# kostas1515/iif

Hardware: AMD Instinct MI355X
Metric: images/sec ResNet50+IIF ImageNet-LT bs=256/GPU (higher is better)
Workload: dtype bf16

## Files before the change

### iif_amd/_lib.py

```python
import ctypes
import os

import torch

_HERE = os.path.dirname(os.path.abspath(__file__))
LIB_PATH = os.environ.get("IIF_AMD_LIB") or os.path.join(_HERE, "csrc", "libiif_amd.so")

IIF_F32, IIF_BF16 = 0, 1
VARIANT_CODE = {"raw": 0, "smooth": 1, "rel": 2, "normit": 3, "gombit": 4, "base2": 5, "base10": 6}
_ERR = {-1: "IIF_EINVAL (bad argument)", -2: "IIF_EUNSUPPORTED (shape/alignment)", -3: "IIF_ELAUNCH (HIP error)"}

_c = ctypes
_P, _I, _L, _F = _c.c_void_p, _c.c_int, _c.c_int64, _c.c_float

SIGNATURES = {
    "iif_build_table": [_P, _I, _I, _I, _P],
    "iif_set_cu_budget": [_I],
    "iif_get_cu_budget": [],
    "iif_ce_fwd_bwd": [_P, _I, _L, _P, _P, _P, _F, _P, _P, _L, _F, _I, _I, _P, _P, _P, _L, _P, _P, _P],
    "iif_sigmoid_focal_fwd_bwd": [_P, _I, _L, _P, _P, _F, _P, _F, _I, _F, _F, _I, _I, _P, _P, _P, _L, _P, _P, _P],
    "iif_scale_logits": [_P, _I, _L, _P, _I, _I, _P, _L, _P],
    "iif_softmax": [_P, _I, _L, _P, _I, _I, _P, _L, _P],
    "iif_topk_hits": [_P, _I, _L, _P, _P, _I, _I, _P, _I, _P, _P],
    "iif_eval_accumulate": [_P, _I, _L, _P, _P, _I, _I, _P, _I, _P, _I, _P, _P, _P, _P],
    "iif_scale_by_device_scalar": [_P, _I, _L, _P, _P, _P],
    "iif_mix_rows": [_P, _I, _P, _F, _I, _L, _P, _P],
    "iif_conv_igemm": [_P, _P, _P, _P, _P, _P, _P],
    "iif_conv_wgrad": [_P, _P, _P, _P, _P, _L, _I, _P],
    "iif_conv_igemm_bnstats": [_P, _P, _P, _P, _P, _P, _P, _L, _P, _P],
    "iif_bn_finalize_stats": [_P, _I, _L, _I, _P, _P, _F, _F, _P, _P, _P, _P, _L, _P],
    "iif_bn_finalize_stats_fused": [_P, _I, _L, _I, _P, _P, _F, _F, _P, _P, _P, _P, _L, _P, _P],
    "iif_bn_finalize_stats_sums": [_P, _I, _L, _I, _P, _P, _F, _F, _P, _P, _P, _P, _L, _P, _P, _I, _I, _P, _P],
    "iif_bn_backward_partials_fused": [_P, _P, _P, _I, _L, _I, _P, _P, _P, _I, _P, _P, _P, _P, _L, _P, _P],
    "iif_bn_partial_sums": [_P, _I, _I, _P, _P],
    "iif_bn_stats_sums": [_P, _I, _L, _I, _P, _P, _L, _P],
    "iif_bn_backward_sums": [_P, _P, _P, _P, _I, _L, _I, _P, _P, _P, _L, _P],
    "iif_bn_backward_apply_sums": [_P, _P, _P, _P, _I, _L, _I, _P, _P, _P, _P, _c.c_double, _P, _P, _P, _P, _P, _P],
    "iif_bn_workspace_bytes": [_L, _I],
    "iif_bn_forward_stats": [_P, _I, _L, _I, _P, _P, _F, _F, _P, _P, _P, _P, _L, _P],
    "iif_bn_apply": [_P, _I, _L, _I, _P, _P, _P, _I, _P, _P, _P],
    "iif_bn_backward": [_P, _P, _P, _P, _I, _L, _I, _P, _P, _P, _P, _P, _P, _P, _L, _P],
    "iif_maxpool_forward": [_P, _I, _I, _I, _I, _I, _I, _I, _I, _P, _P, _P],
    "iif_maxpool_backward": [_P, _P, _I, _I, _I, _I, _I, _I, _I, _I, _P, _P],
# ... 179 lines not shown
```

### iif_amd/csrc/conv_wgrad.hip

```cpp
#include <stdlib.h>
#include <type_traits>

#include "common.h"
#ifndef IIF_WG_AUX_X
#define IIF_WG_AUX_X 0
#endif
#ifndef IIF_WG_AUX_Y
#define IIF_WG_AUX_Y 0
#endif

namespace {

struct WgArgs {
    const unsigned char* x; const unsigned char* dy; float* out;
    int N, Hs, Ws, Cs, Hd, Wd, Cd, R, S, sshift, pad, ldw, M, K;
    int ktiles, ntiles, steps_per_split, nsteps, nsplits;
    int xpitch, ypitch, groups;
    int64_t slab;
};

template <typename T> struct WT;
template <> struct WT<unsigned short> {
    static constexpr int PE = 8, ROWS = 32;
    static constexpr int pitch(int cols) { return cols * 2 + 32; }
// ... 421 lines not shown
}

struct W1Args {
    const unsigned char* x; const unsigned char* dy; float* out;
    int M, Cs, Cd, ldw, ktiles, ntiles, steps_per_split, nsteps, nsplits;
    int64_t slab;
    const unsigned char* dy2; int Cd1, Cd2;
};

template <int OFF> __device__ __forceinline__ s16x4 tr_read_at(unsigned a) {
    s16x4 v;
    asm volatile("ds_read_b64_tr_b16 %0, %1 offset:%2" : "=v"(v) : "v"(a), "n"(OFF) : "memory");
    return v;
}

template <int BC, int BNW, int NWV>
__device__ __forceinline__ void wgrad1x1_body(const W1Args& a, unsigned x_bytes, unsigned dy_bytes) {
    constexpr int NWN = BNW / 64, WK = NWV / NWN, CW = BC / WK, KJ = CW / 16;
    using SX = Swz<unsigned short, BNW>;
    using SY = Swz<unsigned short, BC>;
    constexpr int RBX = SX::RB, RBY = SY::RB;
    constexpr int XB = 32 * RBX, YB = 32 * RBY, STAGE = XB + YB;
    constexpr int NPX = XB / 1024, NPY = YB / 1024;
    constexpr bool YPAD = NPY < NWV;
    constexpr int NIX = NPX / NWV, NIY = YPAD ? 1 : NPY / NWV, LPS = NIX + NIY;
    constexpr int LPRX = RBX / 16, RPIX = 64 / LPRX, LPRY = RBY / 16, RPIY = 64 / LPRY;
    constexpr unsigned OOB = 0xfffffff0u;
    static_assert(NIX >= 1 && NIY >= 1 && NIX * NWV == NPX && (YPAD || NIY * NWV == NPY) && KJ >= 1, "tile geometry");
    static_assert(2 * STAGE + 16 * RBY < 65536 && 2 * STAGE + 16 * RBX < 65536, "fragment reads use 16-bit immediates");
    __shared__ __attribute__((aligned(1024))) unsigned char smem[3 * STAGE + (YPAD ? 1024 : 0)];

    const int tid = threadIdx.x, lane = tid & 63;
// ... 13 lines not shown
    const bool second = a.dy2 != nullptr && k0 >= a.Cd1;
    const int ycols = a.dy2 == nullptr ? a.Cd : (second ? a.Cd2 : a.Cd1);
    const int yk0 = second ? k0 - a.Cd1 : k0;
    const auto rs_y = __builtin_amdgcn_make_buffer_rsrc(const_cast<unsigned char*>(second ? a.dy2 : a.dy), 0,
                                                        second ? (unsigned)a.M * (unsigned)a.Cd2 * 2u : dy_bytes, 0x00020000);

    unsigned offx[NIX], incx[NIX], offy[NIY], incy[NIY];
#pragma unroll
    for (int i = 0; i < NIX; ++i) {
        const int r = RPIX * (NIX * wave + i) + lane / LPRX;
        const int col = n0 + SX::logical(lane % LPRX, r) * 8;
        const bool ok = col < a.Cs;
        offx[i] = ok ? ((unsigned)(step0 * 32 + r) * (unsigned)a.Cs + (unsigned)col) * 2u : OOB;
        incx[i] = ok ? 64u * (unsigned)a.Cs : 0u;
    }
#pragma unroll
    for (int i = 0; i < NIY; ++i) {
        const int r = RPIY * (NIY * wave + i) + lane / LPRY;
        const int col = yk0 + SY::logical(lane % LPRY, r) * 8;
        const bool ok = col < ycols && (!YPAD || wave < NPY);
        offy[i] = ok ? ((unsigned)(step0 * 32 + r) * (unsigned)ycols + (unsigned)col) * 2u : OOB;
        incy[i] = ok ? 64u * (unsigned)ycols : 0u;
    }
    auto issue = [&](auto stage_c) {
        constexpr int S = decltype(stage_c)::value;
#pragma unroll
        for (int i = 0; i < NIX; ++i) {
            __builtin_amdgcn_raw_ptr_buffer_load_lds(rs_x, (lds_void_w*)(smem + S * STAGE + (NIX * wave + i) * 1024), 16, offx[i], 0, 0, IIF_WG_AUX_X);
            offx[i] += incx[i];
        }
#pragma unroll
        for (int i = 0; i < NIY; ++i) {
            unsigned char* dst = smem + S * STAGE + XB + (NIY * wave + i) * 1024;
            if (YPAD && wave >= NPY) dst = smem + 3 * STAGE;
            __builtin_amdgcn_raw_ptr_buffer_load_lds(rs_y, (lds_void_w*)dst, 16, offy[i], 0, 0, IIF_WG_AUX_Y);
            offy[i] += incy[i];
        }
    };

    const int g = lane >> 4, li = lane & 15, q = li >> 2, pp = li & 3;
    unsigned xo[4], yo[KJ];
    const unsigned sbase = (unsigned)(unsigned long long)(lds_cu8*)smem;
#pragma unroll
    for (int ni = 0; ni < 4; ++ni) xo[ni] = sbase + (unsigned)SX::addr(4 * g + q, (wn * 64 + ni * 16 + 4 * pp) * 2);
// ... 52 lines not shown
        const int k = k0 + wk * CW + kj * 16 + li;
        if (k >= a.Cd) continue;
#pragma unroll
        for (int ni = 0; ni < 4; ++ni) {
            const int n = n0 + wn * 64 + ni * 16 + g * 4;
            if (n >= a.Cs) continue;
            *reinterpret_cast<f32x4*>(out + (int64_t)k * a.ldw + n) = acc[ni][kj];
        }
    }
}

__global__ void __launch_bounds__(512) wgrad1x1_256x128_kernel(W1Args a, unsigned xb, unsigned yb) { wgrad1x1_body<256, 128, 8>(a, xb, yb); }
__global__ void __launch_bounds__(256) wgrad1x1_128x128_kernel(W1Args a, unsigned xb, unsigned yb) { wgrad1x1_body<128, 128, 4>(a, xb, yb); }
__global__ void __launch_bounds__(256) wgrad1x1_64x128_kernel(W1Args a, unsigned xb, unsigned yb) { wgrad1x1_body<64, 128, 4>(a, xb, yb); }
__global__ void __launch_bounds__(256) wgrad1x1_64x64_kernel(W1Args a, unsigned xb, unsigned yb) { wgrad1x1_body<64, 64, 4>(a, xb, yb); }
__global__ void __launch_bounds__(512) wgrad1x1_64x256_kernel(W1Args a, unsigned xb, unsigned yb) { wgrad1x1_body<64, 256, 8>(a, xb, yb); }

struct WgHaloArgs {
    const unsigned char* x; const unsigned char* dy; float* out;
    int N, H, W, Cs, Cd, ldw;
    int ci_tiles, co_tiles, steps_per_split, nsteps, nsplits, HB;
    int grouped;
    int64_t slab;
};

template <int XB, int YB, int D>
__global__ void __launch_bounds__(256) conv3x3_wgrad_halo_kernel(WgHaloArgs a, unsigned x_bytes, unsigned dy_bytes) {
    constexpr int RB = 128;
    constexpr int XR = 32 * XB, YR = 32 * YB;
    constexpr unsigned OOB = 0xfffffff0u;
// ... 118 lines not shown
    }
#endif

    float* out = a.out + (int64_t)split * a.slab;
#pragma unroll
    for (int kj = 0; kj < 4; ++kj) {
        const int k = co0 + kj * 16 + li;
#pragma unroll
        for (int tap = 0; tap < 9; ++tap) {
            const int n = a.grouped ? tap * 64 + wave * 16 + g * 4 : tap * a.Cs + ci0 + wave * 16 + g * 4;
            *reinterpret_cast<f32x4*>(out + (int64_t)k * a.ldw + n) = acc[tap][kj];
        }
    }
}

struct WgStemArgs {
    const unsigned char* x; const unsigned char* dy; float* out;
    int N, H, W, ldw, steps_per_split, nsteps, nsplits, LB, LEAD;
    int64_t slab;
};

__global__ void __launch_bounds__(256) conv4x4_s2d_wgrad_kernel(WgStemArgs a, unsigned x_bytes, unsigned dy_bytes) {
    constexpr int XRB = 32, YRB = 128;
    constexpr int XR = 512, YR = 128;
    constexpr int D = 2;
    constexpr unsigned OOB = 0xfffffff0u;
    using SW = Swz<unsigned short, 64>;
    __shared__ __attribute__((aligned(1024))) unsigned char smem[XR * XRB + YR * YRB];
    unsigned char* const XS = smem;
    unsigned char* const YS = smem + XR * XRB;
// ... 182 lines not shown
    if (splits < 1) splits = 1;
    if (splits > h.nsteps) splits = h.nsteps;
    if (splits > 65535) splits = 65535;
    h.steps_per_split = (h.nsteps + splits - 1) / splits;
    splits = (h.nsteps + h.steps_per_split - 1) / h.steps_per_split;
    h.slab = splits > 1 ? slab : 0;
    h.out = splits > 1 ? ws : dw;
    h.nsplits = splits;
    const dim3 grid((unsigned)(tiles * ((splits + 7) / 8) * 8));
    hipLaunchKernelGGL((conv3x3_wgrad_halo_kernel<8, 4, 2>), grid, dim3(256), 0, st, h, (unsigned)x_bytes, (unsigned)dy_bytes);
    IIF_LAUNCH_CHECK();
    if (splits > 1) return reduce_slabs(ws, ws_bytes, splits, slab, a.groups * a.Cd, a.ldw, a.K, dw, st);
    return IIF_OK;
}

inline int launch_wgrad_stem(const WgArgs& a, float* dw, float* ws, int64_t ws_bytes, int splits_req, int64_t x_bytes,
                             int64_t dy_bytes, hipStream_t st) {
    WgStemArgs h{};
    h.x = a.x; h.dy = a.dy; h.N = a.N; h.H = a.Hd; h.W = a.Wd; h.ldw = a.ldw;
    const int Wp = a.Wd + 3;
    h.LB = (2 * Wp + 2 + 31) / 32;
    h.LEAD = h.LB + (31 + Wp + 1) / 32;
    if (h.LEAD + 2 > 14) return -100;
    const int64_t vt = (int64_t)a.N * (a.Hd + 3) * Wp;
    if (vt > 0x7fff0000LL) return -100;
    h.nsteps = (int)((vt + 31) / 32);
    int splits = splits_req;
    if (splits <= 0) {
        const int per_cu = 2;
        splits = 256 * per_cu / share_of(splits_req);
        const int max_by_work = h.nsteps / 8 > 0 ? h.nsteps / 8 : 1;
        if (splits > max_by_work) splits = max_by_work;
    }
    const int64_t slab = (int64_t)a.Cd * a.ldw;
    const int64_t fit = ws ? ws_bytes / (slab * 4) : 0;
    if (splits > fit) splits = (int)fit;
    if (splits < 1) splits = 1;
    if (splits > h.nsteps) splits = h.nsteps;
    if (splits > 65535) splits = 65535;
    h.steps_per_split = (h.nsteps + splits - 1) / splits;
    splits = (h.nsteps + h.steps_per_split - 1) / h.steps_per_split;
    h.slab = splits > 1 ? slab : 0;
    h.out = splits > 1 ? ws : dw;
    h.nsplits = splits;
    hipLaunchKernelGGL(conv4x4_s2d_wgrad_kernel, dim3((unsigned)(((splits + 7) / 8) * 8)), dim3(256), 0, st, h, (unsigned)x_bytes,
                       (unsigned)dy_bytes);
    IIF_LAUNCH_CHECK();
    if (splits > 1) return reduce_slabs(ws, ws_bytes, splits, slab, a.Cd, a.ldw, a.K, dw, st);
    return IIF_OK;
}

inline int launch_wgrad_1x1(const WgArgs& g, float* dw, float* ws, int64_t ws_bytes, int splits_req, int64_t x_bytes, int64_t dy_bytes,
                            hipStream_t st, const unsigned char* dy2 = nullptr, int cd2 = 0) {
    W1Args a{};
    a.x = g.x; a.dy = g.dy; a.M = g.M; a.Cs = g.Cs; a.Cd = g.Cd; a.ldw = g.ldw;
    a.dy2 = dy2; a.Cd1 = dy2 ? g.Cd - cd2 : g.Cd; a.Cd2 = cd2;
    const int bc = dy2 ? (a.Cd1 % 256 == 0 ? 256 : 128) : ((g.Cd >= 256 && g.Cd % 256 == 0) ? 256 : (g.Cd <= 64 ? 64 : 128));
    static const bool no_wide = getenv("IIF_WGRAD_NO_64X256") != nullptr;
    const int bnw = (g.Cs <= 64 && bc == 64) ? 64 : ((bc == 64 && g.Cs > 128 && g.Cs % 256 == 0 && !no_wide) ? 256 : 128);
    a.ktiles = (g.Cd + bc - 1) / bc;
    a.ntiles = (g.Cs + bnw - 1) / bnw;
    a.nsteps = (g.M + 31) / 32;
    const int tiles = a.ktiles * a.ntiles;
    const int per_cu = bc == 256 ? 1 : (bc == 128 ? 3 : (bnw == 256 ? 2 : 4));
    int splits = splits_req;
    const int64_t slab = (int64_t)g.Cd * g.ldw;
    if (splits <= 0) {
        splits = 256 * per_cu / share_of(splits_req) / tiles;
        if (splits < 1) splits = 1;
        const int max_by_work = a.nsteps / 8 > 0 ? a.nsteps / 8 : 1;
        if (splits > max_by_work) splits = max_by_work;
        static const int small_div = [] { const char* e = getenv("IIF_WGRAD_SMALL_DIV"); return e ? atoi(e) : 2; }();
        static const int gram_div = [] { const char* e = getenv("IIF_WGRAD_GRAM_DIV"); return e ? atoi(e) : 8; }();
        const bool gram = g.x == g.dy && dy2 == nullptr;
        static const int small_kb = [] { const char* e = getenv("IIF_WGRAD_SMALL_KB"); return e ? atoi(e) : 256; }();
        static const int mid_div = [] { const char* e = getenv("IIF_WGRAD_MID_DIV"); return e ? atoi(e) : 2; }();
        const int div = gram ? gram_div : (slab * 4 <= ((int64_t)small_kb << 10) ? small_div : (slab * 4 <= (4 << 20) ? mid_div : 1));
        if (div > 1 && splits > 8) { splits /= div; if (splits < 8) splits = 8; }
    }
    const int64_t fit = ws ? ws_bytes / (slab * 4) : 0;
    if (splits > fit) splits = (int)fit;
    if (splits < 1) splits = 1;
    if (splits > a.nsteps) splits = a.nsteps > 0 ? a.nsteps : 1;
    if (splits > 65535) splits = 65535;
    a.steps_per_split = (a.nsteps + splits - 1) / splits;
    splits = (a.nsteps + a.steps_per_split - 1) / a.steps_per_split;
    if (splits < 1) splits = 1;
    a.slab = splits > 1 ? slab : 0;
    a.out = splits > 1 ? ws : dw;
    a.nsplits = splits;
    const dim3 grid((unsigned)(tiles * ((splits + 7) / 8) * 8));
    const unsigned xb = (unsigned)x_bytes, yb = (unsigned)dy_bytes;
    if (bc == 256) hipLaunchKernelGGL(wgrad1x1_256x128_kernel, grid, dim3(512), 0, st, a, xb, yb);
    else if (bc == 128) hipLaunchKernelGGL(wgrad1x1_128x128_kernel, grid, dim3(256), 0, st, a, xb, yb);
    else if (bnw == 256) hipLaunchKernelGGL(wgrad1x1_64x256_kernel, grid, dim3(512), 0, st, a, xb, yb);
    else if (bnw == 128) hipLaunchKernelGGL(wgrad1x1_64x128_kernel, grid, dim3(256), 0, st, a, xb, yb);
    else hipLaunchKernelGGL(wgrad1x1_64x64_kernel, grid, dim3(256), 0, st, a, xb, yb);
    IIF_LAUNCH_CHECK();
    if (splits > 1) return reduce_slabs(ws, ws_bytes, splits, slab, g.Cd, g.ldw, g.Cs, dw, st);
    return IIF_OK;
}

template <typename T>
int launch_wgrad(WgArgs a, float* dw, float* ws, int64_t ws_bytes, int splits_req, int64_t x_bytes, int64_t dy_bytes,
                 hipStream_t st) {
    constexpr int ROWS = WT<T>::ROWS;
    const bool force_v1 = getenv("IIF_CONV_REGSTAGE") != nullptr;
    const bool dma_ok = !force_v1 && x_bytes < 0x7ffffff0LL && dy_bytes < 0x7ffffff0LL;
    if constexpr (sizeof(T) == 2) {
        const bool shape = a.groups == 1 ? (a.Cs % 64 == 0 && a.Cd % 64 == 0 && a.xpitch == a.Cs && a.ypitch == a.Cd)
                                         : (a.Cs == 64 && a.Cd == 64 && a.ldw >= 576);
        const bool halo = dma_ok && shape && a.R == 3 && a.S == 3 && a.sshift == 0 && a.pad == 1 && a.Hs == a.Hd &&
                          a.Ws == a.Wd && a.Wd + 3 <= 64;
        if (halo) {
            const int rc = launch_wgrad_halo(a, dw, ws, ws_bytes, splits_req, x_bytes, dy_bytes, st);
            if (rc != -100) return rc;
        }
        const bool stem = dma_ok && a.groups == 1 && a.R == 4 && a.S == 4 && a.sshift == 0 && a.pad == 2 && a.Hs == a.Hd &&
                          a.Ws == a.Wd && a.Cs == 16 && a.Cd == 64 && a.xpitch == 16 && a.ypitch == 64;
        if (stem) {
            const int rc = launch_wgrad_stem(a, dw, ws, ws_bytes, splits_req, x_bytes, dy_bytes, st);
            if (rc != -100) return rc;
        }
    }
    if constexpr (sizeof(T) == 2) {
        if (dma_ok && a.R == 1 && a.S == 1 && a.sshift == 0 && a.pad == 0 && a.groups == 1 && a.Hs == a.Hd && a.Ws == a.Wd &&
            a.xpitch == a.Cs && a.ypitch == a.Cd)
            return launch_wgrad_1x1(a, dw, ws, ws_bytes, splits_req, x_bytes, dy_bytes, st);
    }
    bool wide = sizeof(T) == 2 && dma_ok && a.groups == 1 && a.Cd >= 256 && a.Cd % 256 == 0;
    const int bc = wide ? 256 : (a.Cd <= 64 ? 64 : 128);
    a.ktiles = (a.Cd + bc - 1) / bc;
    a.ntiles = (a.K + 127) / 128;
    a.nsteps = (a.M + ROWS - 1) / ROWS;
    const int tiles = a.ktiles * a.ntiles;
    int splits = splits_req;
    if (splits <= 0) {
        const int slots = 256 * (bc == 256 ? 1 : (bc == 128 ? 3 : 4)) / share_of(splits_req);
        splits = slots / (tiles * a.groups);
        if (splits < 1) splits = 1;
        const int max_by_work = a.nsteps / 8 > 0 ? a.nsteps / 8 : 1;
        if (splits > max_by_work) splits = max_by_work;
    }
// ... 19 lines not shown
        if (bc == 64) hipLaunchKernelGGL((conv_wgrad_dma_kernel<T, 64>), grid1d, dim3(256), 0, st, a, xb, yb);
        else if (bc == 256) {
            if constexpr (sizeof(T) == 2) hipLaunchKernelGGL((conv_wgrad_dma_kernel<T, 256, 4>), grid1d, dim3(512), 0, st, a, xb, yb);
        } else hipLaunchKernelGGL((conv_wgrad_dma_kernel<T, 128>), grid1d, dim3(256), 0, st, a, xb, yb);
    } else {
        if (bc == 64) hipLaunchKernelGGL((conv_wgrad_kernel<T, 64>), grid, dim3(256), 0, st, a);
        else hipLaunchKernelGGL((conv_wgrad_kernel<T, 128>), grid, dim3(256), 0, st, a);
    }
    IIF_LAUNCH_CHECK();
    if (splits > 1) return reduce_slabs(ws, ws_bytes, splits, slab, a.groups * a.Cd, a.ldw, a.K, dw, st);
    return IIF_OK;
}

}

extern "C" int iif_conv_wgrad(const iif_conv_desc* d, const void* x, const void* dy, float* dw, void* workspace,
                              int64_t workspace_bytes, int splits, void* stream) {
    if (!d || !x || !dy || !dw) return IIF_EINVAL;
    if (d->n <= 0 || d->hs <= 0 || d->ws <= 0 || d->cs <= 0 || d->hd <= 0 || d->wd <= 0 || d->cd <= 0 ||
        d->r <= 0 || d->s <= 0 || d->pad < 0 || workspace_bytes < 0)
        return IIF_EINVAL;
    if (d->stride != 1 && d->stride != 2) return IIF_EUNSUPPORTED;
    if (d->dtype != IIF_F32 && d->dtype != IIF_BF16) return IIF_EINVAL;
    if (d->transposed) return IIF_EINVAL;
    const int pe = d->dtype == IIF_F32 ? 4 : 8;
    if (d->cs % pe != 0 || d->cd % pe != 0 || d->ldw % 4 != 0 || d->ldw < d->r * d->s * d->cs) return IIF_EUNSUPPORTED;
    if ((reinterpret_cast<uintptr_t>(x) | reinterpret_cast<uintptr_t>(dy) | reinterpret_cast<uintptr_t>(dw) |
         reinterpret_cast<uintptr_t>(workspace)) & 15)
        return IIF_EUNSUPPORTED;
    const int64_t M = (int64_t)d->n * d->hd * d->wd;
    if (M > 0x7fffff00LL || (int64_t)d->n * d->hs * d->ws > 0x7fffff00LL) return IIF_EUNSUPPORTED;
    WgArgs a{};
    a.x = (const unsigned char*)x; a.dy = (const unsigned char*)dy;
    a.N = d->n; a.Hs = d->hs; a.Ws = d->ws; a.Cs = d->cs; a.Hd = d->hd; a.Wd = d->wd; a.Cd = d->cd;
    a.R = d->r; a.S = d->s; a.sshift = d->stride - 1; a.pad = d->pad; a.ldw = d->ldw; a.M = (int)M;
    a.K = d->r * d->s * d->cs;
    a.groups = d->groups > 1 ? d->groups : 1;
    a.xpitch = a.groups * d->cs; a.ypitch = a.groups * d->cd;
    if (a.groups > 65535) return IIF_EUNSUPPORTED;
    hipStream_t st = as_stream(stream);
    const int64_t esz = d->dtype == IIF_F32 ? 4 : 2;
    const int64_t x_bytes = (int64_t)d->n * d->hs * d->ws * a.xpitch * esz, dy_bytes = M * a.ypitch * esz;
    if (d->dtype == IIF_BF16)
        return launch_wgrad<unsigned short>(a, dw, (float*)workspace, workspace_bytes, splits, x_bytes, dy_bytes, st);
    return launch_wgrad<float>(a, dw, (float*)workspace, workspace_bytes, splits, x_bytes, dy_bytes, st);
}

extern "C" int iif_wgrad1x1_stacked(const void* x, const void* dy, const void* dy2, int64_t m, int cs, int cd1, int cd2, int ldw,
                                    float* out, void* workspace, int64_t workspace_bytes, int splits, void* stream) {
    if (!x || !dy || !dy2 || !out || m <= 0 || cs <= 0 || cd1 <= 0 || cd2 <= 0 || workspace_bytes < 0) return IIF_EINVAL;
    if (cs % 8 || cd1 % 128 || cd2 % 8 || ldw % 4 || ldw < cs) return IIF_EUNSUPPORTED;
    if ((reinterpret_cast<uintptr_t>(x) | reinterpret_cast<uintptr_t>(dy) | reinterpret_cast<uintptr_t>(dy2) |
         reinterpret_cast<uintptr_t>(out) | reinterpret_cast<uintptr_t>(workspace)) & 15)
        return IIF_EUNSUPPORTED;
    if (m > 0x7fffff00LL || m * cs * 2 >= 0x7f000000LL || m * cd1 * 2 >= 0x7f000000LL || m * cd2 * 2 >= 0x7f000000LL) return IIF_EUNSUPPORTED;
    WgArgs a{};
    a.x = (const unsigned char*)x; a.dy = (const unsigned char*)dy;
// ... 21 lines not shown
```

### iif_amd/ops.py

```python
import ctypes

import torch

from . import _lib
from ._lib import ConvDesc, check, dtype_code, lib, ptr, require_gpu, stream_ptr


def _desc(n, hs, ws, cs, hd, wd, cd, r, s, stride, pad, transposed, ldw, dtype, dst_dtype, groups=1, w_frag=None):
    kind = 0
    if isinstance(w_frag, tuple):
        w_frag, kind = w_frag
    return ConvDesc(n, hs, ws, cs, hd, wd, cd, r, s, stride, pad, transposed, ldw, dtype, dst_dtype, groups,
                    ptr(w_frag) if w_frag is not None else None, kind)


def conv_out_hw(h, w, r, s, stride, pad):
    return (h + 2 * pad - r) // stride + 1, (w + 2 * pad - s) // stride + 1


def conv_forward(x, w, r, s, stride, pad, out=None, out_dtype=None, bias=None, res=None, groups=1, out_hw=None, w_frag=None):
    require_gpu(x, w, bias, res)
    n, h, wd_, cin = x.shape
    cout, ldw = w.shape
    ho, wo = out_hw or conv_out_hw(h, wd_, r, s, stride, pad)
# ... 88 lines not shown
    n, ho, wo, cout = dy.shape
    cin, ldw = wt.shape
    h, w_ = in_hw
    if out is None:
        out = torch.empty((n, h, w_, cin), dtype=dy.dtype, device=dy.device)
    d = _desc(n, ho, wo, cout // groups, h, w_, cin // groups, r, s, stride, pad, 1, ldw, dtype_code(dy), dtype_code(out),
              groups, w_frag)
    if res_bits is not None:
        check(lib().iif_conv_igemm_masked_res(ctypes.byref(d), ptr(dy), ptr(wt), ptr(out), ptr(res), ptr(res_bits),
                                              stream_ptr()), "iif_conv_igemm_masked_res")
        return out
    check(lib().iif_conv_igemm(ctypes.byref(d), ptr(dy), ptr(wt), ptr(out), ptr(res), 0, stream_ptr()), "iif_conv_igemm(dgrad)")
    return out


def conv_wgrad(x, dy, r, s, stride, pad, ldw=None, out=None, workspace=None, splits=0, groups=1):
    require_gpu(x, dy, out, workspace)
    n, h, w_, cin = x.shape
    _, ho, wo, cout = dy.shape
    k = r * s * (cin // groups)
    ldw = ldw or k
    if out is None:
        out = torch.zeros((cout, ldw), dtype=torch.float32, device=x.device)
    elif not out.is_contiguous() or out.numel() < cout * ldw:
        raise ValueError("conv_wgrad: out must be a contiguous float32 [Cout, ldw] tensor (rows are written with pitch ldw)")
    d = _desc(n, h, w_, cin // groups, ho, wo, cout // groups, r, s, stride, pad, 0, ldw, dtype_code(x), _lib.IIF_F32, groups)
    wsb = 0 if workspace is None else workspace.numel() * workspace.element_size()
    check(lib().iif_conv_wgrad(ctypes.byref(d), ptr(x), ptr(dy), ptr(out), ptr(workspace), wsb, splits, stream_ptr()),
          "iif_conv_wgrad")
    return out
# ... 532 lines not shown
```

### include/iif_amd.h

```cpp
#ifndef IIF_AMD_H
#define IIF_AMD_H

#include <stdint.h>

#ifdef __cplusplus
extern "C" {
#endif

#define IIF_OK 0
#define IIF_EINVAL (-1)
#define IIF_EUNSUPPORTED (-2)
#define IIF_ELAUNCH (-3)

#define IIF_F32 0
#define IIF_BF16 1

#define IIF_RAW 0
#define IIF_SMOOTH 1
#define IIF_REL 2
#define IIF_NORMIT 3
#define IIF_GOMBIT 4
#define IIF_BASE2 5
#define IIF_BASE10 6

// ... 112 lines not shown
    int32_t dst_dtype;
    int32_t groups;
    const void* wgt_frag;
    int32_t wgt_frag_kind;
} iif_conv_desc;

int iif_conv_igemm(const iif_conv_desc* d, const void* src, const void* wgt, void* dst,
                   const void* res, const float* bias, void* stream);

int iif_conv_igemm_bnstats(const iif_conv_desc* d, const void* src, const void* wgt, void* dst,
                           const void* res, const float* bias, float* bn_partial,
                           int64_t bn_partial_floats, int32_t* n_partials, void* stream);

int iif_conv_wgrad(const iif_conv_desc* d, const void* x, const void* dy, float* dw,
                   void* workspace, int64_t workspace_bytes, int splits, void* stream);

int iif_wgrad1x1_stacked(const void* x, const void* dy, const void* dy2, int64_t m, int cs, int cd1, int cd2,
                         int ldw, float* out, void* workspace, int64_t workspace_bytes, int splits,
                         void* stream);

int64_t iif_bn_workspace_bytes(int64_t m, int c);
int iif_bn_forward_stats(const void* x, int dtype, int64_t m, int c, const float* gamma,
                         const float* beta, float eps, float momentum, float* running_mean,
                         float* running_var, float* stats, void* workspace,
                         int64_t workspace_bytes, void* stream);
int iif_bn_apply(const void* x, int dtype, int64_t m, int c, const float* stats,
                 const void* residual, const float* residual_stats, int relu, void* y,
                 uint8_t* relu_bits, void* stream);
typedef struct iif_bn_fold_desc {
    const float* gamma; const float* beta; const float* running_mean; const float* running_var;
// ... 299 lines not shown
```

Before: 15290.

## Add specialized stride-2 weight-gradient kernels for 1x1 and 3x3 convolutions

Adds two new weight-gradient paths for stride-2 convolutions, which previously fell back to the general kernel. The 1x1 path is a gather variant of the 1x1 kernel that walks strided input positions incrementally. The 3x3 path uses a ring buffer over parity planes so the nine taps share LDS data and feed MFMA. It also factors routing into a wgrad_family function with a query API, adding kernel complexity and new edge-case logic for odd spatial sizes.

```diff
diff --git a/iif_amd/_lib.py b/iif_amd/_lib.py
--- a/iif_amd/_lib.py
+++ b/iif_amd/_lib.py
@@ -27,6 +27,7 @@
     "iif_mix_rows": [_P, _I, _P, _F, _I, _L, _P, _P],
     "iif_conv_igemm": [_P, _P, _P, _P, _P, _P, _P],
     "iif_conv_wgrad": [_P, _P, _P, _P, _P, _L, _I, _P],
+    "iif_conv_wgrad_route": [_P],
     "iif_conv_igemm_bnstats": [_P, _P, _P, _P, _P, _P, _P, _L, _P, _P],
     "iif_bn_finalize_stats": [_P, _I, _L, _I, _P, _P, _F, _F, _P, _P, _P, _P, _L, _P],
     "iif_bn_finalize_stats_fused": [_P, _I, _L, _I, _P, _P, _F, _F, _P, _P, _P, _P, _L, _P, _P],
diff --git a/iif_amd/csrc/conv_wgrad.hip b/iif_amd/csrc/conv_wgrad.hip
--- a/iif_amd/csrc/conv_wgrad.hip
+++ b/iif_amd/csrc/conv_wgrad.hip
@@ -459,8 +459,10 @@
     return v;
 }
 
-template <int BC, int BNW, int NWV>
-__device__ __forceinline__ void wgrad1x1_body(const W1Args& a, unsigned x_bytes, unsigned dy_bytes) {
+struct W1Gather { int N, Hs, Ws, Hd, Wd; };
+
+template <int BC, int BNW, int NWV, bool GATHER = false>
+__device__ __forceinline__ void wgrad1x1_body(const W1Args& a, unsigned x_bytes, unsigned dy_bytes, const W1Gather& z = W1Gather{}) {
     constexpr int NWN = BNW / 64, WK = NWV / NWN, CW = BC / WK, KJ = CW / 16;
     using SX = Swz<unsigned short, BNW>;
     using SY = Swz<unsigned short, BC>;
@@ -504,6 +506,29 @@
         offx[i] = ok ? ((unsigned)(step0 * 32 + r) * (unsigned)a.Cs + (unsigned)col) * 2u : OOB;
         incx[i] = ok ? 64u * (unsigned)a.Cs : 0u;
     }
+    int gn[NIX], gh[NIX], gw[NIX];
+    bool gok[NIX];
+    int g_rw = 0, g_rh = 0, g_dn = 0;
+    unsigned g_k0 = 0, g_kc = 0, g_kr = 0;
+    if constexpr (GATHER) {
+        const int dq = 32 / z.Wd;
+        g_rw = 32 - dq * z.Wd; g_rh = dq % z.Hd; g_dn = dq / z.Hd;
+        const unsigned colb = 4u * (unsigned)a.Cs, rowb = colb * (unsigned)z.Ws, imgb = 2u * (unsigned)a.Cs * (unsigned)z.Hs * (unsigned)z.Ws;
+        g_k0 = (unsigned)g_rw * colb + (unsigned)g_rh * rowb + (unsigned)g_dn * imgb;
+        g_kc = rowb - (unsigned)z.Wd * colb;
+        g_kr = imgb - (unsigned)z.Hd * rowb;
+#pragma unroll
+        for (int i = 0; i < NIX; ++i) {
+            const int r = RPIX * (NIX * wave + i) + lane / LPRX;
+            const int col = n0 + SX::logical(lane % LPRX, r) * 8;
+            gok[i] = col < a.Cs;
+            const int m = step0 * 32 + r, hw = z.Hd * z.Wd;
+            gn[i] = m / hw;
+            const int rem = m - gn[i] * hw;
+            gh[i] = rem / z.Wd; gw[i] = rem - gh[i] * z.Wd;
+            offx[i] = (((unsigned)(gn[i] * z.Hs + 2 * gh[i]) * (unsigned)z.Ws + 2u * (unsigned)gw[i]) * (unsigned)a.Cs + (unsigned)col) * 2u;
+        }
+    }
 #pragma unroll
     for (int i = 0; i < NIY; ++i) {
         const int r = RPIY * (NIY * wave + i) + lane / LPRY;
@@ -516,8 +541,21 @@
         constexpr int S = decltype(stage_c)::value;
 #pragma unroll
         for (int i = 0; i < NIX; ++i) {
-            __builtin_amdgcn_raw_ptr_buffer_load_lds(rs_x, (lds_void_w*)(smem + S * STAGE + (NIX * wave + i) * 1024), 16, offx[i], 0, 0, IIF_WG_AUX_X);
-            offx[i] += incx[i];
+            if constexpr (GATHER) {
+                const unsigned off = (gok[i] && gn[i] < z.N) ? offx[i] : OOB;
+                __builtin_amdgcn_raw_ptr_buffer_load_lds(rs_x, (lds_void_w*)(smem + S * STAGE + (NIX * wave + i) * 1024), 16, off, 0, 0, IIF_WG_AUX_X);
+                gw[i] += g_rw;
+                const bool c = gw[i] >= z.Wd;
+                gw[i] -= c ? z.Wd : 0;
+                gh[i] += g_rh + (c ? 1 : 0);
+                const bool c2 = gh[i] >= z.Hd;
+                gh[i] -= c2 ? z.Hd : 0;
+                gn[i] += g_dn + (c2 ? 1 : 0);
+                offx[i] += g_k0 + (c ? g_kc : 0u) + (c2 ? g_kr : 0u);
+            } else {
+                __builtin_amdgcn_raw_ptr_buffer_load_lds(rs_x, (lds_void_w*)(smem + S * STAGE + (NIX * wave + i) * 1024), 16, offx[i], 0, 0, IIF_WG_AUX_X);
+                offx[i] += incx[i];
+            }
         }
 #pragma unroll
         for (int i = 0; i < NIY; ++i) {
@@ -600,6 +638,8 @@
 __global__ void __launch_bounds__(256) wgrad1x1_128x128_kernel(W1Args a, unsigned xb, unsigned yb) { wgrad1x1_body<128, 128, 4>(a, xb, yb); }
 __global__ void __launch_bounds__(256) wgrad1x1_64x128_kernel(W1Args a, unsigned xb, unsigned yb) { wgrad1x1_body<64, 128, 4>(a, xb, yb); }
 __global__ void __launch_bounds__(256) wgrad1x1_64x64_kernel(W1Args a, unsigned xb, unsigned yb) { wgrad1x1_body<64, 64, 4>(a, xb, yb); }
+__global__ void __launch_bounds__(512) wgrad1x1s2_256x128_kernel(W1Args a, W1Gather z, unsigned xb, unsigned yb) { wgrad1x1_body<256, 128, 8, true>(a, xb, yb, z); }
+__global__ void __launch_bounds__(256) wgrad1x1s2_128x128_kernel(W1Args a, W1Gather z, unsigned xb, unsigned yb) { wgrad1x1_body<128, 128, 4, true>(a, xb, yb, z); }
 __global__ void __launch_bounds__(512) wgrad1x1_64x256_kernel(W1Args a, unsigned xb, unsigned yb) { wgrad1x1_body<64, 256, 8>(a, xb, yb); }
 
 struct WgHaloArgs {
@@ -748,6 +788,151 @@
     }
 }
 
+struct WgS2Args {
+    const unsigned char* x; const unsigned char* dy; float* out;
+    int N, H, W, Ho, Wo, Cs, Cd, ldw;
+    int ci_tiles, co_tiles, steps_per_split, nsteps, nsplits, LEAD;
+    int64_t slab;
+};
+
+template <int XB, int YB, int D>
+__device__ __forceinline__ void conv3x3s2_wgrad_body(const WgS2Args& a, unsigned x_bytes, unsigned dy_bytes) {
+    constexpr int RB = 128;
+    constexpr int XR = 32 * XB, YR = 32 * YB;
+    constexpr unsigned OOB = 0xfffffff0u;
+    using SW = Swz<unsigned short, 64>;
+    static_assert(D >= 1 && D + 2 <= YB && D + 3 <= XB && (3 * XR + 2 * YR) * RB <= 160 * 1024, "ring geometry");
+    __shared__ __attribute__((aligned(1024))) unsigned char smem[(3 * XR + 2 * YR) * RB];
+    unsigned char* const P11 = smem + 3 * XR * RB;
+    unsigned char* const YS = P11 + YR * RB;
+
+    const int tid = threadIdx.x, lane = tid & 63;
+    const int wave = __builtin_amdgcn_readfirstlane(tid >> 6);
+    const int tiles = a.ci_tiles * a.co_tiles;
+    const int xcd = blockIdx.x & 7, jj = blockIdx.x >> 3;
+    const int split = (jj / tiles) * 8 + xcd, tile = jj % tiles;
+    if (split >= a.nsplits) return;
+    const int ci0 = (tile % a.ci_tiles) * 64, co0 = (tile / a.ci_tiles) * 64;
+    const int step0 = split * a.steps_per_split;
+    int step1 = step0 + a.steps_per_split;
+    if (step1 > a.nsteps) step1 = a.nsteps;
+    const int nst = step1 - step0;
+    const int GH = a.Ho + 1, GW = a.Wo + 1, PV = GH * GW;
+
+    const auto rs_x = __builtin_amdgcn_make_buffer_rsrc(const_cast<unsigned char*>(a.x), 0, x_bytes, 0x00020000);
+    const auto rs_y = __builtin_amdgcn_make_buffer_rsrc(const_cast<unsigned char*>(a.dy), 0, dy_bytes, 0x00020000);
+
+    const int lrow = 8 * wave + (lane >> 3);
+    const unsigned chunk = (unsigned)SW::logical(lane & 7, lrow) * 16u;
+    struct Cur { int n, i, j; };
+    const int dq = 32 / GW, rw = 32 - dq * GW, rh = dq % GH, dn = dq / GH;
+    auto start = [&](int v) {
+        Cur c; c.n = v / PV; const int rem = v - c.n * PV; c.i = rem / GW; c.j = rem - c.i * GW;
+        return c;
+    };
+    auto advance = [&](Cur& c) {
+        c.j += rw;
+        const bool k1 = c.j >= GW;
+        c.j -= k1 ? GW : 0;
+        c.i += rh + (k1 ? 1 : 0);
+        const bool k2 = c.i >= GH;
+        c.i -= k2 ? GH : 0;
+        c.n += dn + (k2 ? 1 : 0);
+    };
+    Cur cx = start(step0 * 32 + lrow), cy = cx;
+    int xblk = 0, yblk = 0;
+    const unsigned xcol = (unsigned)ci0 * 2u + chunk, ycol = (unsigned)co0 * 2u + chunk;
+    auto xoff = [&](const Cur& c, int yy, int xx) {
+        const bool ok = c.n < a.N && (unsigned)yy < (unsigned)a.H && (unsigned)xx < (unsigned)a.W;
+        return ok ? (unsigned)((c.n * a.H + yy) * a.W + xx) * (unsigned)a.Cs * 2u + xcol : OOB;
+    };
+    auto issue_x = [&]() {
+        unsigned char* dst = smem + ((xblk * 32 + 8 * wave) & (XR - 1)) * RB;
+        const int y0 = 2 * cx.i - 1, x0 = 2 * cx.j - 1;
+        __builtin_amdgcn_raw_ptr_buffer_load_lds(rs_x, (lds_void_w*)dst, 16, xoff(cx, y0, x0), 0, 0, IIF_WG_AUX_X);
+        __builtin_amdgcn_raw_ptr_buffer_load_lds(rs_x, (lds_void_w*)(dst + XR * RB), 16, xoff(cx, y0, x0 + 1), 0, 0, IIF_WG_AUX_X);
+        __builtin_amdgcn_raw_ptr_buffer_load_lds(rs_x, (lds_void_w*)(dst + 2 * XR * RB), 16, xoff(cx, y0 + 1, x0), 0, 0, IIF_WG_AUX_X);
+        advance(cx); ++xblk;
+    };
+    auto issue_y = [&]() {
+        const int slot = ((yblk * 32 + 8 * wave) & (YR - 1)) * RB;
+        __builtin_amdgcn_raw_ptr_buffer_load_lds(rs_x, (lds_void_w*)(P11 + slot), 16, xoff(cy, 2 * cy.i, 2 * cy.j), 0, 0, IIF_WG_AUX_X);
+        const bool ok = cy.n < a.N && cy.i < a.Ho && cy.j < a.Wo;
+        const unsigned off = ok ? (unsigned)((cy.n * a.Ho + cy.i) * a.Wo + cy.j) * (unsigned)a.Cd * 2u + ycol : OOB;
+        __builtin_amdgcn_raw_ptr_buffer_load_lds(rs_y, (lds_void_w*)(YS + slot), 16, off, 0, 0, IIF_WG_AUX_Y);
+        advance(cy); ++yblk;
+    };
+
+    f32x4 acc[9][4];
+#pragma unroll
+    for (int t = 0; t < 9; ++t)
+#pragma unroll
+        for (int kj = 0; kj < 4; ++kj) acc[t][kj] = f32x4{0.f, 0.f, 0.f, 0.f};
+
+    for (int j = 0; j < a.LEAD; ++j) issue_x();
+#pragma unroll
+    for (int j = 0; j < D; ++j) { issue_x(); issue_y(); }
+
+    const int g = lane >> 4, li = lane & 15, q = li >> 2, p = li & 3;
+    int xo[9], yo[4];
+#pragma unroll
+    for (int tap = 0; tap < 9; ++tap) {
+        const int r = tap / 3, s_ = tap % 3, plane = (r & 1) * 2 + (s_ & 1), rows = plane == 3 ? YR : XR;
+        xo[tap] = SW::addr((4 * g + q + (r >> 1) * GW + (s_ >> 1)) & (rows - 1), (16 * wave + 4 * p) * 2);
+    }
+#pragma unroll
+    for (int kj = 0; kj < 4; ++kj) yo[kj] = SW::addr(4 * g + q, (16 * kj + 4 * p) * 2);
+    for (int t = 0; t < nst; ++t) {
+        asm volatile("s_waitcnt vmcnt(%0)" ::"n"(5 * (D - 1)) : "memory");
+        __builtin_amdgcn_s_barrier();
+        issue_x(); issue_y();
+        const int ts = t * (32 * RB);
+        TrPair yp[4], xp[9];
+        s16x8 yf[4];
+#pragma unroll
+        for (int kj = 0; kj < 4; ++kj) {
+            yp[kj].lo = tr_read(YS + ((yo[kj] + ts) & (YR * RB - 1))); yp[kj].hi = tr_read(YS + ((yo[kj] + ts + 16 * RB) & (YR * RB - 1)));
+        }
+#pragma unroll
+        for (int tap = 0; tap < 9; ++tap) {
+            const int plane = ((tap / 3) & 1) * 2 + ((tap % 3) & 1);
+            const int mask = (plane == 3 ? YR : XR) * RB - 1;
+            const unsigned char* ring = smem + plane * XR * RB;
+            xp[tap].lo = tr_read(ring + ((xo[tap] + ts) & mask)); xp[tap].hi = tr_read(ring + ((xo[tap] + ts + 16 * RB) & mask));
+        }
+#pragma unroll
+        for (int tap = 0; tap < 9; ++tap) {
+            if (tap == 0) tr_fence<15>(); else if (tap == 1) tr_fence<14>(); else if (tap == 2) tr_fence<12>();
+            else if (tap == 3) tr_fence<10>(); else if (tap == 4) tr_fence<8>(); else if (tap == 5) tr_fence<6>();
+            else if (tap == 6) tr_fence<4>(); else if (tap == 7) tr_fence<2>(); else tr_fence<0>();
+            if (tap == 0) {
+#pragma unroll
+                for (int kj = 0; kj < 4; ++kj) yf[kj] = tr_join(yp[kj]);
+            }
+            const s16x8 xf = tr_join(xp[tap]);
+#pragma unroll
+            for (int kj = 0; kj < 4; ++kj)
+                acc[tap][kj] = __builtin_amdgcn_mfma_f32_16x16x32_bf16(__builtin_bit_cast(bf16x8, xf), __builtin_bit_cast(bf16x8, yf[kj]),
+                                                                        acc[tap][kj], 0, 0, 0);
+        }
+    }
+    asm volatile("s_waitcnt vmcnt(0)" ::: "memory");
+
+    float* out = a.out + (int64_t)split * a.slab;
+#pragma unroll
+    for (int kj = 0; kj < 4; ++kj) {
+        const int k = co0 + kj * 16 + li;
+#pragma unroll
+        for (int tap = 0; tap < 9; ++tap) {
+            const int n = tap * a.Cs + ci0 + wave * 16 + g * 4;
+            *reinterpret_cast<f32x4*>(out + (int64_t)k * a.ldw + n) = acc[tap][kj];
+        }
+    }
+}
+
+__global__ void __launch_bounds__(256) conv3x3s2_wgrad_deep_kernel(WgS2Args a, unsigned xb, unsigned yb) { conv3x3s2_wgrad_body<8, 4, 2>(a, xb, yb); }
+__global__ void __launch_bounds__(256) conv3x3s2_wgrad_shallow_kernel(WgS2Args a, unsigned xb, unsigned yb) { conv3x3s2_wgrad_body<4, 4, 1>(a, xb, yb); }
+
 struct WgStemArgs {
     const unsigned char* x; const unsigned char* dy; float* out;
     int N, H, W, ldw, steps_per_split, nsteps, nsplits, LB, LEAD;
@@ -960,6 +1145,11 @@
     return IIF_OK;
 }
 
+inline bool stem_fits(const WgArgs& a) {
+    const int Wp = a.Wd + 3;
+    const int lead = (2 * Wp + 2 + 31) / 32 + (31 + Wp + 1) / 32;
+    return lead + 2 <= 14 && (int64_t)a.N * (a.Hd + 3) * Wp <= 0x7fff0000LL;
+}
 inline int launch_wgrad_stem(const WgArgs& a, float* dw, float* ws, int64_t ws_bytes, int splits_req, int64_t x_bytes,
                              int64_t dy_bytes, hipStream_t st) {
     WgStemArgs h{};
@@ -967,9 +1157,8 @@
     const int Wp = a.Wd + 3;
     h.LB = (2 * Wp + 2 + 31) / 32;
     h.LEAD = h.LB + (31 + Wp + 1) / 32;
-    if (h.LEAD + 2 > 14) return -100;
+    if (!stem_fits(a)) return -100;
     const int64_t vt = (int64_t)a.N * (a.Hd + 3) * Wp;
-    if (vt > 0x7fff0000LL) return -100;
     h.nsteps = (int)((vt + 31) / 32);
     int splits = splits_req;
     if (splits <= 0) {
@@ -997,11 +1186,11 @@
 }
 
 inline int launch_wgrad_1x1(const WgArgs& g, float* dw, float* ws, int64_t ws_bytes, int splits_req, int64_t x_bytes, int64_t dy_bytes,
-                            hipStream_t st, const unsigned char* dy2 = nullptr, int cd2 = 0) {
+                            hipStream_t st, const unsigned char* dy2 = nullptr, int cd2 = 0, bool gather = false) {
     W1Args a{};
     a.x = g.x; a.dy = g.dy; a.M = g.M; a.Cs = g.Cs; a.Cd = g.Cd; a.ldw = g.ldw;
     a.dy2 = dy2; a.Cd1 = dy2 ? g.Cd - cd2 : g.Cd; a.Cd2 = cd2;
-    const int bc = dy2 ? (a.Cd1 % 256 == 0 ? 256 : 128) : ((g.Cd >= 256 && g.Cd % 256 == 0) ? 256 : (g.Cd <= 64 ? 64 : 128));
+    const int bc = dy2 ? (a.Cd1 % 256 == 0 ? 256 : 128) : ((g.Cd >= 256 && g.Cd % 256 == 0) ? 256 : ((g.Cd <= 64 && !gather) ? 64 : 128));
     static const bool no_wide = getenv("IIF_WGRAD_NO_64X256") != nullptr;
     const int bnw = (g.Cs <= 64 && bc == 64) ? 64 : ((bc == 64 && g.Cs > 128 && g.Cs % 256 == 0 && !no_wide) ? 256 : 128);
     a.ktiles = (g.Cd + bc - 1) / bc;
@@ -1021,7 +1210,9 @@
         const bool gram = g.x == g.dy && dy2 == nullptr;
         static const int small_kb = [] { const char* e = getenv("IIF_WGRAD_SMALL_KB"); return e ? atoi(e) : 256; }();
         static const int mid_div = [] { const char* e = getenv("IIF_WGRAD_MID_DIV"); return e ? atoi(e) : 2; }();
-        const int div = gram ? gram_div : (slab * 4 <= ((int64_t)small_kb << 10) ? small_div : (slab * 4 <= (4 << 20) ? mid_div : 1));
+        int div = gram ? gram_div : (slab * 4 <= ((int64_t)small_kb << 10) ? small_div : (slab * 4 <= (4 << 20) ? mid_div : 1));
+        static const int gather_div = [] { const char* e = getenv("IIF_WGRAD_S2_DIV"); return e ? atoi(e) : 1; }();
+        if (gather) div = gather_div;
         if (div > 1 && splits > 8) { splits /= div; if (splits < 8) splits = 8; }
     }
     const int64_t fit = ws ? ws_bytes / (slab * 4) : 0;
@@ -1037,7 +1228,11 @@
     a.nsplits = splits;
     const dim3 grid((unsigned)(tiles * ((splits + 7) / 8) * 8));
     const unsigned xb = (unsigned)x_bytes, yb = (unsigned)dy_bytes;
-    if (bc == 256) hipLaunchKernelGGL(wgrad1x1_256x128_kernel, grid, dim3(512), 0, st, a, xb, yb);
+    if (gather) {
+        const W1Gather z{g.N, g.Hs, g.Ws, g.Hd, g.Wd};
+        if (bc == 256) hipLaunchKernelGGL(wgrad1x1s2_256x128_kernel, grid, dim3(512), 0, st, a, z, xb, yb);
+        else hipLaunchKernelGGL(wgrad1x1s2_128x128_kernel, grid, dim3(256), 0, st, a, z, xb, yb);
+    } else if (bc == 256) hipLaunchKernelGGL(wgrad1x1_256x128_kernel, grid, dim3(512), 0, st, a, xb, yb);
     else if (bc == 128) hipLaunchKernelGGL(wgrad1x1_128x128_kernel, grid, dim3(256), 0, st, a, xb, yb);
     else if (bnw == 256) hipLaunchKernelGGL(wgrad1x1_64x256_kernel, grid, dim3(512), 0, st, a, xb, yb);
     else if (bnw == 128) hipLaunchKernelGGL(wgrad1x1_64x128_kernel, grid, dim3(256), 0, st, a, xb, yb);
@@ -1047,6 +1242,72 @@
     return IIF_OK;
 }
 
+inline bool halo_s2_fits(const WgArgs& a) {
+    const int64_t vt = (int64_t)a.N * (a.Hd + 1) * (a.Wd + 1);
+    return 1 + (a.Wd + 1) / 32 <= 4 && vt <= 0x7fff0000LL;
+}
+inline int launch_wgrad_halo_s2(const WgArgs& a, float* dw, float* ws, int64_t ws_bytes, int splits_req, int64_t x_bytes,
+                                int64_t dy_bytes, hipStream_t st) {
+    if (!halo_s2_fits(a)) return -100;
+    WgS2Args h{};
+    h.x = a.x; h.dy = a.dy; h.N = a.N; h.H = a.Hs; h.W = a.Ws; h.Ho = a.Hd; h.Wo = a.Wd; h.Cs = a.Cs; h.Cd = a.Cd; h.ldw = a.ldw;
+    h.ci_tiles = a.Cs / 64; h.co_tiles = a.Cd / 64;
+    h.LEAD = 1 + (a.Wd + 1) / 32;
+    const int64_t vt = (int64_t)a.N * (a.Hd + 1) * (a.Wd + 1);
+    h.nsteps = (int)((vt + 31) / 32);
+    const int tiles = h.ci_tiles * h.co_tiles;
+    const char* e = getenv("IIF_WGRAD_S2_RINGS");
+    const bool shallow = h.LEAD == 1 && !(e && e[0] == 'd');
+    int splits = splits_req;
+    if (splits <= 0) {
+        const int per_cu = shallow ? 2 : 1;
+        splits = 256 * per_cu / share_of(splits_req) / tiles;
+        if (splits < 1) splits = 1;
+        const int max_by_work = h.nsteps / 8 > 0 ? h.nsteps / 8 : 1;
+        if (splits > max_by_work) splits = max_by_work;
+    }
+    const int64_t slab = (int64_t)a.Cd * a.ldw;
+    const int64_t fit = ws ? ws_bytes / (slab * 4) : 0;
+    if (splits > fit) splits = (int)fit;
+    if (splits < 1) splits = 1;
+    if (splits > h.nsteps) splits = h.nsteps;
+    if (splits > 65535) splits = 65535;
+    h.steps_per_split = (h.nsteps + splits - 1) / splits;
+    splits = (h.nsteps + h.steps_per_split - 1) / h.steps_per_split;
+    h.slab = splits > 1 ? slab : 0;
+    h.out = splits > 1 ? ws : dw;
+    h.nsplits = splits;
+    const dim3 grid((unsigned)(tiles * ((splits + 7) / 8) * 8));
+    if (shallow) hipLaunchKernelGGL(conv3x3s2_wgrad_shallow_kernel, grid, dim3(256), 0, st, h, (unsigned)x_bytes, (unsigned)dy_bytes);
+    else hipLaunchKernelGGL(conv3x3s2_wgrad_deep_kernel, grid, dim3(256), 0, st, h, (unsigned)x_bytes, (unsigned)dy_bytes);
+    IIF_LAUNCH_CHECK();
+    if (splits > 1) return reduce_slabs(ws, ws_bytes, splits, slab, a.Cd, a.ldw, a.K, dw, st);
+    return IIF_OK;
+}
+
+inline int wgrad_family(const WgArgs& a, int esz, int64_t x_bytes, int64_t dy_bytes) {
+    const bool force_v1 = getenv("IIF_CONV_REGSTAGE") != nullptr;
+    const bool dma_ok = !force_v1 && x_bytes < 0x7ffffff0LL && dy_bytes < 0x7ffffff0LL;
+    if (esz != 2 || !dma_ok) return IIF_WGRAD_GENERAL;
+    const bool same_grid = a.sshift == 0 && a.Hs == a.Hd && a.Ws == a.Wd;
+    const bool half_grid = a.sshift == 1 && getenv("IIF_WGRAD_NO_S2") == nullptr;
+    const bool dense64 = a.groups == 1 && a.Cs % 64 == 0 && a.Cd % 64 == 0 && a.xpitch == a.Cs && a.ypitch == a.Cd;
+    const bool shape = a.groups == 1 ? dense64 : (a.Cs == 64 && a.Cd == 64 && a.ldw >= 576);
+    if (shape && a.R == 3 && a.S == 3 && same_grid && a.pad == 1 && a.Wd + 3 <= 64 &&
+        (int64_t)a.N * (a.Hd + 2) * (a.Wd + 2) <= 0x7fff0000LL)
+        return IIF_WGRAD_NINETAP;
+    if (a.groups == 1 && a.R == 4 && a.S == 4 && same_grid && a.pad == 2 && a.Cs == 16 && a.Cd == 64 && a.xpitch == 16 && a.ypitch == 64 &&
+        stem_fits(a))
+        return IIF_WGRAD_STEM;
+    if (a.R == 1 && a.S == 1 && same_grid && a.pad == 0 && a.groups == 1 && a.xpitch == a.Cs && a.ypitch == a.Cd) return IIF_WGRAD_1X1;
+    if (half_grid && dense64 && a.R == 1 && a.S == 1 && a.pad == 0 && a.Hd == (a.Hs - 1) / 2 + 1 && a.Wd == (a.Ws - 1) / 2 + 1)
+        return IIF_WGRAD_1X1_S2;
+    if (half_grid && dense64 && a.R == 3 && a.S == 3 && a.pad == 1 && a.Hd == (a.Hs - 1) / 2 + 1 && a.Wd == (a.Ws - 1) / 2 + 1 &&
+        halo_s2_fits(a))
+        return IIF_WGRAD_NINETAP_S2;
+    return IIF_WGRAD_GENERAL;
+}
+
 template <typename T>
 int launch_wgrad(WgArgs a, float* dw, float* ws, int64_t ws_bytes, int splits_req, int64_t x_bytes, int64_t dy_bytes,
                  hipStream_t st) {
@@ -1054,25 +1315,16 @@
     const bool force_v1 = getenv("IIF_CONV_REGSTAGE") != nullptr;
     const bool dma_ok = !force_v1 && x_bytes < 0x7ffffff0LL && dy_bytes < 0x7ffffff0LL;
     if constexpr (sizeof(T) == 2) {
-        const bool shape = a.groups == 1 ? (a.Cs % 64 == 0 && a.Cd % 64 == 0 && a.xpitch == a.Cs && a.ypitch == a.Cd)
-                                         : (a.Cs == 64 && a.Cd == 64 && a.ldw >= 576);
-        const bool halo = dma_ok && shape && a.R == 3 && a.S == 3 && a.sshift == 0 && a.pad == 1 && a.Hs == a.Hd &&
-                          a.Ws == a.Wd && a.Wd + 3 <= 64;
-        if (halo) {
-            const int rc = launch_wgrad_halo(a, dw, ws, ws_bytes, splits_req, x_bytes, dy_bytes, st);
-            if (rc != -100) return rc;
-        }
-        const bool stem = dma_ok && a.groups == 1 && a.R == 4 && a.S == 4 && a.sshift == 0 && a.pad == 2 && a.Hs == a.Hd &&
-                          a.Ws == a.Wd && a.Cs == 16 && a.Cd == 64 && a.xpitch == 16 && a.ypitch == 64;
-        if (stem) {
-            const int rc = launch_wgrad_stem(a, dw, ws, ws_bytes, splits_req, x_bytes, dy_bytes, st);
-            if (rc != -100) return rc;
-        }
-    }
-    if constexpr (sizeof(T) == 2) {
-        if (dma_ok && a.R == 1 && a.S == 1 && a.sshift == 0 && a.pad == 0 && a.groups == 1 && a.Hs == a.Hd && a.Ws == a.Wd &&
-            a.xpitch == a.Cs && a.ypitch == a.Cd)
-            return launch_wgrad_1x1(a, dw, ws, ws_bytes, splits_req, x_bytes, dy_bytes, st);
+        int rc = -100;
+        switch (wgrad_family(a, 2, x_bytes, dy_bytes)) {
+        case IIF_WGRAD_NINETAP: rc = launch_wgrad_halo(a, dw, ws, ws_bytes, splits_req, x_bytes, dy_bytes, st); break;
+        case IIF_WGRAD_STEM: rc = launch_wgrad_stem(a, dw, ws, ws_bytes, splits_req, x_bytes, dy_bytes, st); break;
+        case IIF_WGRAD_1X1: return launch_wgrad_1x1(a, dw, ws, ws_bytes, splits_req, x_bytes, dy_bytes, st);
+        case IIF_WGRAD_1X1_S2: return launch_wgrad_1x1(a, dw, ws, ws_bytes, splits_req, x_bytes, dy_bytes, st, nullptr, 0, true);
+        case IIF_WGRAD_NINETAP_S2: rc = launch_wgrad_halo_s2(a, dw, ws, ws_bytes, splits_req, x_bytes, dy_bytes, st); break;
+        default: break;
+        }
+        if (rc != -100) return rc;
     }
     bool wide = sizeof(T) == 2 && dma_ok && a.groups == 1 && a.Cd >= 256 && a.Cd % 256 == 0;
     const int bc = wide ? 256 : (a.Cd <= 64 ? 64 : 128);
@@ -1122,33 +1374,51 @@
 
 }
 
-extern "C" int iif_conv_wgrad(const iif_conv_desc* d, const void* x, const void* dy, float* dw, void* workspace,
-                              int64_t workspace_bytes, int splits, void* stream) {
-    if (!d || !x || !dy || !dw) return IIF_EINVAL;
+static int wgrad_args(const iif_conv_desc* d, WgArgs* out, int64_t* x_bytes, int64_t* dy_bytes) {
     if (d->n <= 0 || d->hs <= 0 || d->ws <= 0 || d->cs <= 0 || d->hd <= 0 || d->wd <= 0 || d->cd <= 0 ||
-        d->r <= 0 || d->s <= 0 || d->pad < 0 || workspace_bytes < 0)
+        d->r <= 0 || d->s <= 0 || d->pad < 0)
         return IIF_EINVAL;
     if (d->stride != 1 && d->stride != 2) return IIF_EUNSUPPORTED;
     if (d->dtype != IIF_F32 && d->dtype != IIF_BF16) return IIF_EINVAL;
     if (d->transposed) return IIF_EINVAL;
     const int pe = d->dtype == IIF_F32 ? 4 : 8;
     if (d->cs % pe != 0 || d->cd % pe != 0 || d->ldw % 4 != 0 || d->ldw < d->r * d->s * d->cs) return IIF_EUNSUPPORTED;
-    if ((reinterpret_cast<uintptr_t>(x) | reinterpret_cast<uintptr_t>(dy) | reinterpret_cast<uintptr_t>(dw) |
-         reinterpret_cast<uintptr_t>(workspace)) & 15)
-        return IIF_EUNSUPPORTED;
     const int64_t M = (int64_t)d->n * d->hd * d->wd;
     if (M > 0x7fffff00LL || (int64_t)d->n * d->hs * d->ws > 0x7fffff00LL) return IIF_EUNSUPPORTED;
     WgArgs a{};
-    a.x = (const unsigned char*)x; a.dy = (const unsigned char*)dy;
     a.N = d->n; a.Hs = d->hs; a.Ws = d->ws; a.Cs = d->cs; a.Hd = d->hd; a.Wd = d->wd; a.Cd = d->cd;
     a.R = d->r; a.S = d->s; a.sshift = d->stride - 1; a.pad = d->pad; a.ldw = d->ldw; a.M = (int)M;
     a.K = d->r * d->s * d->cs;
     a.groups = d->groups > 1 ? d->groups : 1;
     a.xpitch = a.groups * d->cs; a.ypitch = a.groups * d->cd;
     if (a.groups > 65535) return IIF_EUNSUPPORTED;
+    const int64_t esz = d->dtype == IIF_F32 ? 4 : 2;
+    *x_bytes = (int64_t)d->n * d->hs * d->ws * a.xpitch * esz; *dy_bytes = M * a.ypitch * esz;
+    *out = a;
+    return IIF_OK;
+}
+
+extern "C" int iif_conv_wgrad_route(const iif_conv_desc* d) {
+    if (!d) return IIF_EINVAL;
+    WgArgs a{};
+    int64_t x_bytes = 0, dy_bytes = 0;
+    const int rc = wgrad_args(d, &a, &x_bytes, &dy_bytes);
+    if (rc != IIF_OK) return rc;
+    return wgrad_family(a, d->dtype == IIF_F32 ? 4 : 2, x_bytes, dy_bytes);
+}
+
+extern "C" int iif_conv_wgrad(const iif_conv_desc* d, const void* x, const void* dy, float* dw, void* workspace,
+                              int64_t workspace_bytes, int splits, void* stream) {
+    if (!d || !x || !dy || !dw || workspace_bytes < 0) return IIF_EINVAL;
+    WgArgs a{};
+    int64_t x_bytes = 0, dy_bytes = 0;
+    const int rc = wgrad_args(d, &a, &x_bytes, &dy_bytes);
+    if (rc != IIF_OK) return rc;
+    if ((reinterpret_cast<uintptr_t>(x) | reinterpret_cast<uintptr_t>(dy) | reinterpret_cast<uintptr_t>(dw) |
+         reinterpret_cast<uintptr_t>(workspace)) & 15)
+        return IIF_EUNSUPPORTED;
+    a.x = (const unsigned char*)x; a.dy = (const unsigned char*)dy;
     hipStream_t st = as_stream(stream);
-    const int64_t esz = d->dtype == IIF_F32 ? 4 : 2;
-    const int64_t x_bytes = (int64_t)d->n * d->hs * d->ws * a.xpitch * esz, dy_bytes = M * a.ypitch * esz;
     if (d->dtype == IIF_BF16)
         return launch_wgrad<unsigned short>(a, dw, (float*)workspace, workspace_bytes, splits, x_bytes, dy_bytes, st);
     return launch_wgrad<float>(a, dw, (float*)workspace, workspace_bytes, splits, x_bytes, dy_bytes, st);
diff --git a/iif_amd/ops.py b/iif_amd/ops.py
--- a/iif_amd/ops.py
+++ b/iif_amd/ops.py
@@ -126,6 +126,18 @@
     return out
 
 
+WGRAD_ROUTES = ("general", "ninetap", "stem", "1x1", "1x1_s2", "ninetap_s2")
+
+
+def conv_wgrad_route(n, hs, ws, cs, hd, wd, cd, r, s, stride, pad, ldw, dtype=torch.bfloat16, groups=1):
+    code = _lib.IIF_BF16 if dtype == torch.bfloat16 else _lib.IIF_F32
+    d = _desc(n, hs, ws, cs, hd, wd, cd, r, s, stride, pad, 0, ldw, code, _lib.IIF_F32, groups)
+    rc = lib().iif_conv_wgrad_route(ctypes.byref(d))
+    if rc < 0:
+        check(rc, "iif_conv_wgrad_route")
+    return WGRAD_ROUTES[rc]
+
+
 def conv_wgrad(x, dy, r, s, stride, pad, ldw=None, out=None, workspace=None, splits=0, groups=1):
     require_gpu(x, dy, out, workspace)
     n, h, w_, cin = x.shape
diff --git a/include/iif_amd.h b/include/iif_amd.h
--- a/include/iif_amd.h
+++ b/include/iif_amd.h
@@ -150,6 +150,13 @@
 
 int iif_conv_wgrad(const iif_conv_desc* d, const void* x, const void* dy, float* dw,
                    void* workspace, int64_t workspace_bytes, int splits, void* stream);
+#define IIF_WGRAD_GENERAL 0
+#define IIF_WGRAD_NINETAP 1
+#define IIF_WGRAD_STEM 2
+#define IIF_WGRAD_1X1 3
+#define IIF_WGRAD_1X1_S2 4
+#define IIF_WGRAD_NINETAP_S2 5
+int iif_conv_wgrad_route(const iif_conv_desc* d);
 
 int iif_wgrad1x1_stacked(const void* x, const void* dy, const void* dy2, int64_t m, int cs, int cd1, int cd2,
                          int ldw, float* out, void* workspace, int64_t workspace_bytes, int splits,
```

After: 15420 (median of 6 runs). About the same (+0.9%).
